# huang-yh/GaussianFormer

Measured on AMD Instinct MI355X. Metric: Gaussians/sec splatted into 200×200×16×18 voxel grid (fwd), higher is better.
Workload: dtype f32

## Files before the change

### gaussianformer_amd/csrc/splat_bwd_mfma.hip

```cpp
#include <algorithm>


#include "gf_common.hpp"
#include "splat_mfma.hpp"

#ifndef GF_TIMELINE
#define GF_TIMELINE 0
#endif

namespace gf {

constexpr int kBwdBigTableAt = kLongWords, kBwdBigTable = (kBwdBigCap - kBwdBigTableAt - 1) / 3;
static_assert(kBwdBigTableAt >= kWRow && kBwdBigTable >= 64, "the table sits past the layout words in use");

struct BwdMArgs {
    const float *pts;
    const float *records;
    const uint2 *boxes;
    const unsigned long long *bitmask;
    const float *out_grad;
    float *rows;
    float *means_grad, *opa_grad, *sem_grad, *cov_grad;
    const uint32_t *state;
    uint32_t *tile_counters;
    const uint32_t *gen_word;
    const uint32_t *row_first;
    const uint32_t *wave_total;
    const uint32_t *lists, *list_len;
    const uint32_t *lists_bad;
    int P, N, nwords, nrow, H, W, D, nsx, nsy;
    int gate;
    int records_asserted;
    unsigned long long *timeline;
    uint32_t *big_table;
    uint32_t m_ps, m_nsy;
    uint32_t cap;
};

static_assert(kBwdList == 256, "kMList");
constexpr int kMList = kBwdList;
constexpr int kMQCap = 128;
constexpr int kMPitch16 = 136;
constexpr int kMDlDwords = kC * kMPitch16;
static_assert(128 * kC <= kMDlDwords, "the 128 fp32 rows land in the same area before they are split");
constexpr int kMFirstAt = 1536 + 3 * kMList + kMDlDwords + kMQCap;
constexpr int kMLdsDwords = kMFirstAt + 64;
constexpr int kMRowAt = 768;
static_assert(kMRowAt + 2 * kWRow <= 1536 + 3 * kMList, "the bitmask row fits over the slot's upper half and the list");
static_assert(3 * kMList <= kMRowAt, "the dense-word compaction borrows the lower half of the record slot");
static_assert(kMLdsDwords * 4 <= 20480, "eight single-wave workgroups per CU");

__device__ __forceinline__ void split16(const f32x16 &d, H8 (&hi)[2], H8 (&lo)[2])
{
#pragma unroll
    for (int q = 0; q < 16; q += 2) {
        const float w0 = d[q], w1 = d[q + 1];
        const fp16x2 h = __builtin_amdgcn_cvt_pkrtz(w0, w1);
        float q0, q1;
        asm("v_fma_mix_f32 %0, %1, -1.0, %2 op_sel_hi:[1,0,0]" : "=v"(q0) : "v"(h), "v"(w0));
        asm("v_fma_mix_f32 %0, %1, -1.0, %2 op_sel:[1,0,0] op_sel_hi:[1,0,0]" : "=v"(q1) : "v"(h), "v"(w1));
        hi[q >> 3].p[(q & 7) >> 1] = h;
        lo[q >> 3].p[(q & 7) >> 1] = __builtin_amdgcn_cvt_pkrtz(q0, q1);
    }
}

struct BwdSetupArgs {
    float *means_grad, *opa_grad, *sem_grad, *cov_grad;
    const uint32_t *wave_total, *row_local;
    uint32_t *row_first;
    uint32_t *gen_word;
    const uint32_t *state;
    uint32_t cap;
    int P;
};

__global__ __launch_bounds__(256) void gf_splat_bwd_setup_kernel(BwdSetupArgs a)
{
    if (!on_matrix_cores(a.state[kStateNotDense], a.state[kStatePath])) return;
    if (records_still_there(a.state, a.gen_word)) return;
    const size_t i0 = (size_t)blockIdx.x * 256 + threadIdx.x, stride = (size_t)gridDim.x * 256;
    for (size_t i = i0; i < (size_t)kC * a.P; i += stride) a.sem_grad[i] = 0.f;
    for (size_t i = i0; i < (size_t)6 * a.P; i += stride) a.cov_grad[i] = 0.f;
    for (size_t i = i0; i < (size_t)3 * a.P; i += stride) a.means_grad[i] = 0.f;
    for (size_t i = i0; i < (size_t)a.P; i += stride) a.opa_grad[i] = 0.f;
    const int nblk = (a.P + 255) >> 8;
    if ((int)blockIdx.x >= nblk) return;
    __shared__ uint32_t s_sum[4];
    const int tid = threadIdx.x, w0 = 4 * (int)blockIdx.x, nw = (a.P + 63) >> 6;
    const int g = 256 * (int)blockIdx.x + tid;
    const uint32_t local = g < a.P ? a.row_local[g] : 0u;
    uint32_t before = 0u;
    for (int w = tid; w < w0; w += 256) before += a.wave_total[w] & 0x7FFFFFFFu;
#pragma unroll
    for (int off = 32; off >= 1; off >>= 1) before += (uint32_t)__shfl_xor((int)before, off, 64);
    if ((tid & 63) == 0) s_sum[tid >> 6] = before;
    __syncthreads();
    uint32_t base = s_sum[0] + s_sum[1] + s_sum[2] + s_sum[3];
    const int wv = tid >> 6;
    uint32_t mine = 0u;
    for (int k = 0; k < 4; ++k) {
        const uint32_t t = w0 + k < nw ? (a.wave_total[w0 + k] & 0x7FFFFFFFu) : 0u;
        if (k < wv) base += t;
        if (k == wv) mine = t;
    }
    if (g < a.P) a.row_first[g] = (unsigned long long)base + mine <= (unsigned long long)a.cap ? base + local : 0xFFFFFFFFu;
}

__device__ __forceinline__ void zero_big_gaussians(const BwdMArgs &a, int lane)
{
    const int nw = (a.P + 63) >> 6;
    constexpr int kPer = (kWRow + 63) / 64;
    static_assert(kPer == 10, "operand list below");
    int nbig = 0;
    for (int kb = 0; 64 * kb < nw; kb += kPer) {
    uint32_t fl[kPer];
#pragma unroll
    for (int k = 0; k < kPer; ++k) fl[k] = a.wave_total[min(64 * (kb + k) + lane, nw - 1)];
    asm volatile("" : "+v"(fl[0]), "+v"(fl[1]), "+v"(fl[2]), "+v"(fl[3]), "+v"(fl[4]), "+v"(fl[5]), "+v"(fl[6]), "+v"(fl[7]), "+v"(fl[8]), "+v"(fl[9]));
#pragma unroll
    for (int k = 0; k < kPer; ++k) {
        const int w0 = 64 * (kb + k);
        const bool f = w0 + lane < nw && (fl[k] >> 31) != 0u;
        unsigned long long m = __builtin_amdgcn_ballot_w64(f);
        while (m) {
            const int w = w0 + __builtin_ctzll(m);
            m &= m - 1;
            const int g = 64 * w + lane;
            bool big_here = false;
            uint32_t first_here = 0u;
            int cnt_here = 0;
            if (g < a.P) {
                const uint2 b = a.boxes[g];
                const bool ne = ux(b.y) > ux(b.x) && uy(b.y) > uy(b.x) && uz(b.y) > uz(b.x);
                const int cnt = !ne ? 0 : (((ux(b.y) - 1) >> 2) - (ux(b.x) >> 2) + 1) * (((uy(b.y) - 1) >> 2) - (uy(b.x) >> 2) + 1) *
                                              (((uz(b.y) - 1) >> 3) - (uz(b.x) >> 3) + 1);
                first_here = a.row_first[g];
                if (cnt > kBwdBigRows && first_here != 0xFFFFFFFFu) {
                    for (int k = 0; k < kC; ++k) a.sem_grad[(size_t)kC * g + k] = 0.f;
                    for (int k = 0; k < 6; ++k) a.cov_grad[6 * (size_t)g + k] = 0.f;
                    for (int k = 0; k < 3; ++k) a.means_grad[3 * (size_t)g + k] = 0.f;
                    a.opa_grad[g] = 0.f;
                    big_here = true;
                    cnt_here = cnt;
                }
            }
            const unsigned long long bm = __builtin_amdgcn_ballot_w64(big_here);
            if (big_here) {
                const int pos = nbig + __builtin_popcountll(bm & ((1ull << lane) - 1ull));
                if (pos < kBwdBigTable) {
                    a.big_table[1 + 3 * pos] = (uint32_t)g;
                    a.big_table[2 + 3 * pos] = first_here;
                    a.big_table[3 + 3 * pos] = (uint32_t)cnt_here;
                }
            }
            nbig += __builtin_popcountll(bm);
        }
    }
    }
    if (lane == 0) a.big_table[0] = nbig <= kBwdBigTable ? (uint32_t)nbig : 0xFFFFFFFFu;
}

template <bool LONG = false>
__global__ __launch_bounds__(64, 2) void gf_splat_bwd_mfma_kernel(BwdMArgs a)
{
    __shared__ __attribute__((aligned(16))) uint32_t s_u[kMLdsDwords];
    float4 *slot = reinterpret_cast<float4 *>(s_u);
    uint32_t *s_lg = s_u + 1536, *s_blo = s_u + 1536 + kMList, *s_bhi = s_u + 1536 + 2 * kMList;
    float *s_dl = reinterpret_cast<float *>(s_u + 1536 + 3 * kMList);
    unsigned long long *s_row = reinterpret_cast<unsigned long long *>(s_u + kMRowAt);
    uint32_t *q_id = s_u + 1536 + 3 * kMList + kMDlDwords;
    _Float16 *s_dh = reinterpret_cast<_Float16 *>(s_dl), *s_dq = s_dh + kC * kMPitch16;

    uint32_t st0 = a.state[kStateNotDense], st1 = a.state[kStatePath], st3 = a.state[kStateGen], st4 = a.state[kStateRows], gen = *a.gen_word;
    uint32_t lbad = a.lists ? *a.lists_bad : 1u;
    asm volatile("" : "+s"(st0), "+s"(st1), "+s"(st3), "+s"(st4), "+s"(gen), "+s"(lbad));
    const bool mc_fwd = on_matrix_cores(st0, st1);
    const bool still_there = st3 == gen && (st4 & kRowsReady) != 0u;
    if (a.gate && !mc_fwd) return;
    if (a.records_asserted && !still_there) return;

    const int lane = threadIdx.x;
    if (blockIdx.x == 0) zero_big_gaussians(a, lane);
    const int n_ = lane & 31, h_ = lane >> 5;
    typedef _Float16 half2_t __attribute__((ext_vector_type(2)));
    const int xcd = (int)(blockIdx.x & 7u);
    const int per_super = 4 * ((a.D + 7) >> 3);
    const int per_xcd = ((a.nsx * a.nsy + 7) >> 3) * per_super;
    const uint32_t m_ps = a.m_ps, m_nsy = a.m_nsy;

    cfloat_t cp = (cfloat_t)(uintptr_t)a.pts;
    const double p0x = cp[0], p0y = cp[1], p0z = cp[2];
    const double sx = a.H > 1 ? (double)cp[3 * (size_t)a.W * a.D] - p0x : 1.0;
    const double sy = a.W > 1 ? (double)cp[3 * (size_t)a.D + 1] - p0y : 1.0;
    const double sz = a.D > 1 ? (double)cp[3 + 2] - p0z : 1.0;

    auto request_records_at = [&](int qh, int start, int count) {
        const uint32_t id = q_id[(qh + start + (n_ < count ? n_ : 0)) & (kMQCap - 1)];
        const char *rec = reinterpret_cast<const char *>(a.records + (size_t)id * kRecDwords);
        const int o3 = (3 + 2 * h_) * 16, o4 = (4 + 2 * h_) * 16, o5 = 7 * 16;
        char *dst = reinterpret_cast<char *>(slot);
        __builtin_amdgcn_global_load_lds((gptr)(rec), (lptr)(dst), 16, 0, 0);
        __builtin_amdgcn_global_load_lds((gptr)(rec + 16), (lptr)(dst + 1024), 16, 0, 0);
        __builtin_amdgcn_global_load_lds((gptr)(rec + 32), (lptr)(dst + 2048), 16, 0, 0);
        __builtin_amdgcn_global_load_lds((gptr)(rec + o3), (lptr)(dst + 3072), 16, 0, 0);
        __builtin_amdgcn_global_load_lds((gptr)(rec + o4), (lptr)(dst + 4096), 16, 0, 0);
        __builtin_amdgcn_global_load_lds((gptr)(rec + o5), (lptr)(dst + 5120), 16, 0, 0);
        __builtin_amdgcn_global_load_lds((gptr)(a.row_first + id), (lptr)(s_u + kMFirstAt), 4, 0, 0);
    };
    auto request_row = [&](const unsigned long long *bm, int wl) {
        for (int i = 0; 128 * i < a.nrow; ++i)
            if (128 * i + 2 * wl < a.nrow)
                __builtin_amdgcn_global_load_lds((gptr)(bm + 128 * i + 2 * wl), (lptr)(s_row + 128 * i), 16, 0, 0);
    };

    const bool dl_by16 = (a.D & 1) == 0;
    const size_t dl_last = (size_t)a.N * kC - (dl_by16 ? 4 : 1);
    const bool use_lists = a.lists && still_there && (LONG || lbad == 0u);
    auto request_unit = [&](int s_, int Xw_, int Y0_, int Zw_) {
        int wl = lane;
        asm volatile("" : "+v"(wl));
        if (use_lists) {
            const int pstride = LONG ? kBwdPubLong : kMList;
            const uint32_t *src = a.lists + (size_t)s_ * (3 * pstride) + 4 * wl;
#pragma unroll
            for (int k = 0; k < 3; ++k)
                __builtin_amdgcn_global_load_lds((gptr)(src + pstride * k), (lptr)(s_lg + kMList * k), 16, 0, 0);
        } else if (!LONG) {
            request_row(a.bitmask + (size_t)s_ * a.nrow, wl);
        }
        const int per_col = dl_by16 ? 36 : 144, step_off = dl_by16 ? 28 : 64, step_col = dl_by16 ? 1 : 0, fl = dl_by16 ? 4 : 1;
        int col = wl >= per_col ? 1 : 0, off = wl - col * per_col;
        const int nreq = dl_by16 ? 9 : 36;
#pragma nounroll
        for (int i = 0; i < nreq; ++i) {
            const int cx = Xw_ + (col >> 2), cy = Y0_ + (col & 3);
            const bool ok = cx < a.H && cy < a.W;
            const size_t vox = ok ? ((size_t)cx * a.W + cy) * a.D + Zw_ : 0;
            const size_t fo = min(vox * kC + (size_t)(off * fl), dl_last);
            const float *src = a.out_grad + fo;
            if (dl_by16) __builtin_amdgcn_global_load_lds((gptr)src, (lptr)(s_dl + 256 * i), 16, 0, 0);
            else __builtin_amdgcn_global_load_lds((gptr)src, (lptr)(s_dl + 64 * i), 4, 0, 0);
            col += step_col; off += step_off;
            if (off >= per_col) { off -= per_col; col += 1; }
        }
    };

    uint32_t *ctr = a.tile_counters + 64 * xcd;
    const int nchunk = (a.nwords + 63) >> 6;
    int local = (int)(blockIdx.x >> 3);
    while (true) {
        const int logical = local;
        const int qs = (int)__umulhi((uint32_t)logical, m_ps);
        if (!(local < per_xcd && 8 * qs + xcd < a.nsx * a.nsy)) break;
        uint32_t claimed = 0u;
        const int s = 8 * qs + xcd, r = logical - qs * per_super;
        const int srow = a.nsy == 1 ? s : (int)__umulhi((uint32_t)s, m_nsy), scol = s - srow * a.nsy;
        const int Xw = srow * kSuper + 4 * (r & 1), Y0 = scol * kSuper + 4 * ((r >> 1) & 1), Zw = 8 * (r >> 2);
        if (Xw < a.H && Y0 < a.W) {
#if GF_TIMELINE
            unsigned long long tl[8] = {(unsigned long long)wall_clock64(), 0, 0, 0, 0, 0, 0, 0};
#endif
            const uint32_t published_len = use_lists ? a.list_len[s] : 0u;
            request_unit(s, Xw, Y0, Zw);
            if (dl_by16) asm volatile("s_waitcnt vmcnt(9)" ::: "memory");
            else asm volatile("s_waitcnt vmcnt(36)" ::: "memory");
#if GF_TIMELINE
            tl[1] = wall_clock64();
#endif
            int list_len = 0, qlen = 0, qhead = 0, npend = 0;
            int c = 0, sg = 0;
            bool have_boxes = false;
            const bool pub_unit = LONG ? (use_lists && published_len != 0xFFFFFFFFu) : use_lists;
            int pub_done = 0;
            bool pub_fetch = false;
            if (pub_unit) {
                list_len = min((int)(LONG ? published_len : (published_len & 0xFFFFu)), kMList);
                c = nchunk;
                have_boxes = true;
            } else if (!LONG) {
                constexpr int kWDense = kMList;
                uint32_t *s_dw = s_u;
                unsigned long long *s_db = reinterpret_cast<unsigned long long *>(s_u + kWDense);
                constexpr int kWPer = (kWRow + 63) / 64;
                const int kw = nchunk;
                unsigned long long wd[kWPer];
                int mine = 0;
                int wlane = lane;
                asm volatile("" : "+v"(wlane));
                const int wbase = kw * wlane;
#pragma unroll
                for (int k = 0; k < kWPer; ++k) wd[k] = s_row[min(wbase + k, kWRow - 1)];
                static_assert(kWPer == 10, "operand list below");
                asm volatile("" : "+v"(wd[0]), "+v"(wd[1]), "+v"(wd[2]), "+v"(wd[3]), "+v"(wd[4]), "+v"(wd[5]), "+v"(wd[6]), "+v"(wd[7]),
                             "+v"(wd[8]), "+v"(wd[9]));
#pragma unroll
                for (int k = 0; k < kWPer; ++k) {
                    const int w = wbase + k;
                    wd[k] = (k < kw && w < a.nwords) ? wd[k] : 0ull;
                    mine += wd[k] != 0ull ? 1 : 0;
                }
                const int incl_nz = wave_incl_scan_dpp(mine);
                const int nd = __builtin_amdgcn_readlane(incl_nz, 63);
                if (nd <= kWDense) {
                    int p = incl_nz - mine;
#pragma unroll
                    for (int k = 0; k < kWPer; ++k) {
                        if (wd[k] != 0ull) {
                            s_dw[p] = (uint32_t)(wbase + k);
                            s_db[p] = wd[k];
                            ++p;
                        }
                    }
                    __builtin_amdgcn_fence(__ATOMIC_ACQ_REL, "wavefront");
                    __builtin_amdgcn_wave_barrier();
                    int tot = 0;
                    bool fits = true;
                    auto extract = [&](unsigned long long bits, uint32_t id0, int pos) {
                        if (bits) {
                            s_lg[pos++] = id0 + (uint32_t)__builtin_ctzll(bits);
                            bits &= bits - 1;
                        }
                        while (bits) {
                            const int j = __builtin_ctzll(bits);
                            bits &= bits - 1;
                            s_lg[pos++] = id0 + (uint32_t)j;
                        }
                    };
                    if (nd <= 192) {
                        unsigned long long bb[3];
                        uint32_t ii[3];
                        int cn[3], in_[3], tt[3];
#pragma unroll
                        for (int q = 0; q < 3; ++q) {
                            bb[q] = s_db[64 * q + lane];
                            ii[q] = s_dw[64 * q + lane];
                        }
                        asm volatile("" : "+v"(bb[0]), "+v"(bb[1]), "+v"(bb[2]), "+v"(ii[0]), "+v"(ii[1]), "+v"(ii[2]));
#pragma unroll
                        for (int q = 0; q < 3; ++q) {
                            bb[q] = 64 * q + lane < nd ? bb[q] : 0ull;
                            ii[q] *= 64u;
                            cn[q] = __builtin_popcountll(bb[q]);
                        }
#pragma unroll
                        for (int q = 0; q < 3; ++q) in_[q] = wave_incl_scan_dpp(cn[q]);
#pragma unroll
                        for (int q = 0; q < 3; ++q) tt[q] = __builtin_amdgcn_readlane(in_[q], 63);
                        tot = tt[0] + tt[1] + tt[2];
                        if (tot <= kMList) {
                            extract(bb[0], ii[0], in_[0] - cn[0]);
                            extract(bb[1], ii[1], tt[0] + in_[1] - cn[1]);
                            extract(bb[2], ii[2], tt[0] + tt[1] + in_[2] - cn[2]);
                        } else {
                            fits = false;
                        }
                    } else {
                        for (int d0 = 0; d0 < nd; d0 += 64) {
                            const int i = d0 + lane;
                            const unsigned long long bits = i < nd ? s_db[i] : 0ull;
                            const uint32_t id0 = (i < nd ? s_dw[i] : 0u) * 64u;
                            const int cnt = __builtin_popcountll(bits);
                            const int incl = wave_incl_scan_dpp(cnt);
                            const int t = __builtin_amdgcn_readlane(incl, 63);
                            if (tot + t > kMList) {
                                fits = false;
                                break;
                            }
                            extract(bits, id0, tot + incl - cnt);
                            tot += t;
                        }
                    }
                    if (fits) {
                        list_len = tot;
                        c = nchunk;
                    }
                }
            }
            const unsigned long long *bm_row = a.bitmask + (size_t)s * a.nrow;
#if GF_TIMELINE
            tl[2] = wall_clock64();
#endif
            __builtin_amdgcn_fence(__ATOMIC_ACQ_REL, "wavefront");
            __builtin_amdgcn_wave_barrier();
            asm volatile("s_waitcnt vmcnt(0)" ::: "memory");
            float dmax = 0.f;
            float v[2 * kC];
            {
                int wl = lane;
                asm volatile("" : "+v"(wl));
                const int ly_ = (wl >> 3) & 3, z_ = wl & 7;
#pragma unroll
                for (int half = 0; half < 2; ++half) {
                    const int lx_ = (wl >> 5) + 2 * half;
                    const bool ok = Xw + lx_ < a.H && Y0 + ly_ < a.W && Zw + z_ < a.D;
                    const float *rowp = s_dl + (64 * half + wl) * kC;
                    const float4 q0 = *reinterpret_cast<const float4 *>(rowp), q1 = *reinterpret_cast<const float4 *>(rowp + 4);
                    const float4 q2 = *reinterpret_cast<const float4 *>(rowp + 8), q3 = *reinterpret_cast<const float4 *>(rowp + 12);
                    const float2 q4 = *reinterpret_cast<const float2 *>(rowp + 16);
                    const float w[kC] = {q0.x, q0.y, q0.z, q0.w, q1.x, q1.y, q1.z, q1.w, q2.x, q2.y, q2.z, q2.w, q3.x, q3.y, q3.z, q3.w, q4.x, q4.y};
#pragma unroll
                    for (int ch = 0; ch < kC; ++ch) v[2 * ch + half] = ok ? w[ch] : 0.f;
                }
#pragma unroll
                for (int k = 0; k < 2 * kC; ++k) dmax = fmaxf(dmax, fabsf(v[k]));
#pragma unroll
                for (int d = 32; d >= 1; d >>= 1) dmax = fmaxf(dmax, __shfl_xor(dmax, d, 64));
            }
            const int dex = min(254, max(5, (int)((__float_as_uint(dmax) >> 23) & 255u)));
            const float dscale = dmax > 0.f ? __uint_as_float((uint32_t)(258 - dex) << 23) : 1.f;
            const int dshift = dmax > 0.f ? dex - 131 : 0;
            {
                __builtin_amdgcn_fence(__ATOMIC_ACQ_REL, "wavefront");
                __builtin_amdgcn_wave_barrier();
                int wl = lane;
                asm volatile("" : "+v"(wl));
                const int colv = 32 * (2 * ((wl >> 2) & 1)) + 16 * ((wl >> 5) & 1) + 4 * ((wl >> 3) & 3) + (wl & 3);
                _Float16 *ph = s_dh + colv, *pq = s_dq + colv;
#pragma unroll
                for (int ch = 0; ch < kC; ++ch) {
                    const float x0 = v[2 * ch] * dscale, x1 = v[2 * ch + 1] * dscale;
                    const fp16x2 hh = __builtin_amdgcn_cvt_pkrtz(x0, x1);
                    float q0, q1;
                    asm("v_fma_mix_f32 %0, %1, -1.0, %2 op_sel_hi:[1,0,0]" : "=v"(q0) : "v"(hh), "v"(x0));
                    asm("v_fma_mix_f32 %0, %1, -1.0, %2 op_sel:[1,0,0] op_sel_hi:[1,0,0]" : "=v"(q1) : "v"(hh), "v"(x1));
                    const fp16x2 ll = __builtin_amdgcn_cvt_pkrtz(q0, q1);
                    ph[ch * kMPitch16] = hh[0]; ph[ch * kMPitch16 + 32] = hh[1];
                    pq[ch * kMPitch16] = ll[0]; pq[ch * kMPitch16 + 32] = ll[1];
                }
                __builtin_amdgcn_fence(__ATOMIC_ACQ_REL, "wavefront");
                __builtin_amdgcn_wave_barrier();
            }
            int n = n_, h = h_;
            asm volatile("" : "+v"(n), "+v"(h));
            h8 phi[4], hotv[2];
        #pragma unroll
            for (int b = 0; b < 4; ++b) {
                const float ux_ = (float)(2 * (b & 1) + (n >> 4)) - 1.5f, uy_ = (float)((n >> 2) & 3) - 1.5f,
                            uz_ = (float)(4 * (b >> 1) + (n & 3)) - 3.5f;
                const float m0[8] = {1.f, ux_, uy_, uz_, ux_ * ux_, 0.f, 0.f, 0.f};
                const float m1[8] = {uy_ * uy_, uz_ * uz_, ux_ * uy_, uy_ * uz_, ux_ * uz_, 0.f, 0.f, 0.f};
        #pragma unroll
                for (int j = 0; j < 8; ++j) phi[b][j] = (_Float16)(h ? m1[j] : m0[j]);
            }
        #pragma unroll
            for (int k = 0; k < 2; ++k) {
                const int lx = 2 * k + (n >> 4), ly = (n >> 2) & 3, zz = 4 * k + (n & 3);
        #pragma unroll
                for (int j = 0; j < 8; ++j) hotv[k][j] = (_Float16)((h ? zz == j : (j < 4 ? lx == j : ly == j - 4)) ? 1.f : 0.f);
            }
            
            half2_t xy2[4][2], z2[2][2];
            {
                const int mono = (n & 4) ? -1 : ((n & 3) + 4 * (n >> 3));
                const int pa[10] = {0, 1, 0, 0, 2, 0, 0, 1, 0, 1}, pb[10] = {0, 0, 1, 0, 0, 2, 0, 1, 1, 0}, pc[10] = {0, 0, 0, 1, 0, 0, 2, 0, 1, 1};
                int ea = 0, eb = 0, ec = 0;
        #pragma unroll
                for (int m = 0; m < 10; ++m) {
                    ea = mono == m ? pa[m] : ea; eb = mono == m ? pb[m] : eb; ec = mono == m ? pc[m] : ec;
                }
                const bool valid_row = mono >= 0 && mono < 10;
                auto pw = [](float x, int e) { return e == 0 ? 1.f : (e == 1 ? x : x * x); };
        #pragma unroll
                for (int t = 0; t < 4; ++t)
        #pragma unroll
                    for (int jy = 0; jy < 2; ++jy) {
                        const float v = valid_row ? pw((float)t - 1.5f, ea) * pw((float)(h + 2 * jy) - 1.5f, eb) : 0.f;
                        xy2[t][jy] = (half2_t){(_Float16)v, (_Float16)v};
                    }
        #pragma unroll
                for (int bz = 0; bz < 2; ++bz)
        #pragma unroll
                    for (int zp = 0; zp < 2; ++zp)
                        z2[bz][zp] = (half2_t){(_Float16)pw((float)(4 * bz + 2 * zp) - 3.5f, ec), (_Float16)pw((float)(4 * bz + 2 * zp + 1) - 3.5f, ec)};
            }
            const double Cx = p0x + ((double)Xw + 1.5) * sx, Cy = p0y + ((double)Y0 + 1.5) * sy, Cz = p0z + ((double)Zw + 3.5) * sz;
            bool have_next = false;
            bool stores_behind = false;
#if GF_TIMELINE
            asm volatile("s_waitcnt lgkmcnt(0)" ::: "memory");
            tl[3] = wall_clock64();
#endif
            while (true) {
                bool last = false;
                if (LONG && pub_unit) {
                    if (pub_fetch) {
                        int wl = lane;
                        asm volatile("" : "+v"(wl));
                        const int e0 = min(pub_done + 4 * wl, kBwdPubLong - 4);
                        const uint32_t *src = a.lists + (size_t)s * (3 * kBwdPubLong) + e0;
#pragma unroll
                        for (int k = 0; k < 3; ++k)
                            __builtin_amdgcn_global_load_lds((gptr)(src + kBwdPubLong * k), (lptr)(s_lg + kMList * k), 16, 0, 0);
                        asm volatile("s_waitcnt vmcnt(0)" ::: "memory");
                        list_len = min((int)published_len - pub_done, kMList);
                        have_boxes = true;
                    }
                    pub_done += list_len;
                    last = pub_done >= (int)published_len;
                    pub_fetch = true;
                }
                while (!(LONG && pub_unit)) {
                    if (c >= nchunk) {
                        last = true;
                        break;
                    }
                    const int w = 64 * c + lane;
                    unsigned long long bits = w < a.nwords ? bm_row[w] : 0ull;
                    const int cnt = __builtin_popcountll(bits);
                    const int incl = wave_incl_scan_dpp(cnt);
                    const int total = __builtin_amdgcn_readlane(incl, 63);
                    int pos = -1;
                    if (total <= kMList) {
                        if (list_len + total > kMList) break;
                        pos = list_len + incl - cnt;
                        list_len += total;
                        ++c;
                    } else {
                        static_assert(4 * 64 <= kMList, "a lane group of four words fits the empty list");
                        bool full = false;
                        for (; sg < 16; ++sg) {
                            const int e1 = __builtin_amdgcn_readlane(incl, 4 * sg + 3);
                            const int e0 = sg ? __builtin_amdgcn_readlane(incl, 4 * sg - 1) : 0;
                            if (list_len + (e1 - e0) > kMList) {
                                full = true;
                                break;
                            }
                            if ((lane >> 2) == sg) pos = list_len + (incl - cnt) - e0;
                            list_len += e1 - e0;
                        }
                        if (!full) {
                            sg = 0;
                            ++c;
                        }
                        if (pos >= 0) {
                            const uint32_t id0 = (uint32_t)w * 64u;
                            while (bits) {
                                const int j = __builtin_ctzll(bits);
                                bits &= bits - 1;
                                s_lg[pos++] = id0 + (uint32_t)j;
                            }
                        }
                        if (full) break;
                        continue;
                    }
                    const uint32_t id0 = (uint32_t)w * 64u;
                    while (bits) {
                        const int j = __builtin_ctzll(bits);
                        bits &= bits - 1;
                        s_lg[pos++] = id0 + (uint32_t)j;
                    }
                }
                __builtin_amdgcn_fence(__ATOMIC_ACQ_REL, "wavefront");
                __builtin_amdgcn_wave_barrier();
                if (!have_boxes) {
                    for (int b0 = 0; b0 < list_len; b0 += 64) {
                        const uint32_t id = s_lg[min(b0 + lane, list_len - 1)];
                        __builtin_amdgcn_global_load_lds((gptr)(&a.boxes[id].x), (lptr)(s_blo + b0), 4, 0, 0);
                        __builtin_amdgcn_global_load_lds((gptr)(&a.boxes[id].y), (lptr)(s_bhi + b0), 4, 0, 0);
                    }
                    asm volatile("s_waitcnt vmcnt(0)" ::: "memory");
                }
                have_boxes = false;
                stores_behind = false;
                for (int base = 0; base < list_len || (last && base == 0); base += 64) {
                    const int i = base + lane;
                    const int ic = min(i, max(list_len - 1, 0));
                    const uint32_t eg = s_lg[ic];
                    const uint32_t blo = s_blo[ic], bhi = s_bhi[ic];
                    const bool hit = i < list_len && ux(blo) < Xw + 4 && ux(bhi) > Xw && uy(blo) < Y0 + 4 && uy(bhi) > Y0 &&
                                     uz(blo) < Zw + 8 && uz(bhi) > Zw;
                    const unsigned long long todo = __builtin_amdgcn_ballot_w64(hit);
                    if (hit) q_id[(qhead + qlen + (int)mbcnt(todo)) & (kMQCap - 1)] = eg;
                    qlen += __builtin_popcountll(todo);
                    const bool final_batch = last && base + 64 >= list_len;
                    while (true) {
                        if (npend == 0) {
                            if (!(qlen >= 32 || (final_batch && qlen > 0))) break;
                            npend = min(qlen, 32);
                            __builtin_amdgcn_fence(__ATOMIC_ACQ_REL, "wavefront");
                            __builtin_amdgcn_wave_barrier();
                            request_records_at(qhead, 0, npend);
                            stores_behind = false;
                        }
                        const int avail = qlen - npend;
                        if (!(avail >= 32 || final_batch)) break;
                        const int qn = npend;
                        if (stores_behind) asm volatile("s_waitcnt vmcnt(6)" ::: "memory");
                        else asm volatile("s_waitcnt vmcnt(0)" ::: "memory");
#if GF_TIMELINE
                        if (!tl[4]) tl[4] = wall_clock64();
                        tl[7] += 1;
#endif
                        const bool live = n < qn;
                        const float4 r0 = slot[lane], r1 = slot[64 + lane], r2 = slot[128 + lane];
                        const float4 e0 = slot[192 + lane], e1 = slot[256 + lane], e2 = slot[320 + lane];
                        const uint32_t my_id = q_id[(qhead + (live ? n : 0)) & (kMQCap - 1)];
                        const uint32_t first = s_u[kMFirstAt + lane];
                        __builtin_amdgcn_fence(__ATOMIC_ACQ_REL, "wavefront");
                        __builtin_amdgcn_wave_barrier();
                        const int nnext = min(avail, 32);
                        if (nnext > 0) request_records_at(qhead, qn, nnext);
                        const bool last_group = final_batch && nnext == 0;
                        if (last_group && lane == 0)
                            asm volatile("global_atomic_add %0, %1, %2, off sc0" : "=v"(claimed) : "v"(ctr), "v"(1u) : "memory");
                        H8 b0h, b0l, b1h, b1l;
                        int sshift = 0;
                        {
                            float sv[10] = {e0.x, e0.y, e0.z, e0.w, e1.x, e1.y, e1.z, e1.w, e2.x, e2.y};
                            float smax = 0.f;
#pragma unroll
                            for (int j = 0; j < 10; ++j) {
                                sv[j] = live ? sv[j] : 0.f;
                                smax = fmaxf(smax, fabsf(sv[j]));
                            }
                            smax = fmaxf(smax, __builtin_bit_cast(float, __builtin_amdgcn_ds_bpermute((lane ^ 32) << 2, __builtin_bit_cast(int, smax))));
                            const int sex = min(252, (int)((__float_as_uint(smax) >> 23) & 255u));
                            const float sscale = smax > 0.f ? __uint_as_float((uint32_t)(253 - sex) << 23) : 1.f;
                            sshift = smax > 0.f ? sex - 126 : 0;
#pragma unroll
                            for (int j = 0; j < 10; ++j) sv[j] *= sscale;
                            if (h) { sv[8] = 0.f; sv[9] = 0.f; }
                            const fp16x2 zz = __builtin_amdgcn_cvt_pkrtz(0.f, 0.f);
#pragma unroll
                            for (int j = 0; j < 10; j += 2) {
                                const fp16x2 hh = __builtin_amdgcn_cvt_pkrtz(sv[j], sv[j + 1]);
                                float q0, q1;
                                asm("v_fma_mix_f32 %0, %1, -1.0, %2 op_sel_hi:[1,0,0]" : "=v"(q0) : "v"(hh), "v"(sv[j]));
                                asm("v_fma_mix_f32 %0, %1, -1.0, %2 op_sel:[1,0,0] op_sel_hi:[1,0,0]" : "=v"(q1) : "v"(hh), "v"(sv[j + 1]));
                                const fp16x2 ll = __builtin_amdgcn_cvt_pkrtz(q0, q1);
                                if (j < 8) { b0h.p[j >> 1] = hh; b0l.p[j >> 1] = ll; }
                                else { b1h.p[0] = hh; b1l.p[0] = ll; }
                            }
#pragma unroll
                            for (int j = 1; j < 4; ++j) { b1h.p[j] = zz; b1l.p[j] = zz; }
                            b1h.p[1] = b1l.p[0]; b1h.p[2] = b1h.p[0];
                        }
                        H8 t1, t2, t3;
                        double ex = 0, ey = 0, ez = 0;
                        {
                            const double L = 1.4426950408889634074;
                            const double c0 = r1.x, c1 = r1.y, c2 = r1.z, c3 = r1.w, c4 = r2.x, c5 = r2.y;
                            double th[5];
                            if (h == 0) {
                                ex = Cx - (double)r0.x; ey = Cy - (double)r0.y; ez = Cz - (double)r0.z;
                                const double gx = c0 * ex + c3 * ey + c5 * ez, gy = c3 * ex + c1 * ey + c4 * ez, gz = c5 * ex + c4 * ey + c2 * ez;
                                th[0] = -0.5 * L * (ex * gx + ey * gy + ez * gz);
                                th[1] = -L * sx * gx; th[2] = -L * sy * gy; th[3] = -L * sz * gz;
                                th[4] = -0.5 * L * sx * sx * c0;
                            } else {
                                th[0] = -0.5 * L * sy * sy * c1; th[1] = -0.5 * L * sz * sz * c2;
                                th[2] = -L * sx * sy * c3; th[3] = -L * sy * sz * c4; th[4] = -L * sx * sz * c5;
                            }
#pragma unroll
                            for (int j = 0; j < 5; ++j) split3(live ? th[j] : 0.0, t1.e[j], t2.e[j], t3.e[j]);
#pragma unroll
                            for (int j = 5; j < 8; ++j) { t1.e[j] = (_Float16)0.f; t2.e[j] = (_Float16)0.f; t3.e[j] = (_Float16)0.f; }
                        }
                        H8 tb;
                        {
                            const uint32_t glo = __float_as_uint(r2.z), ghi = __float_as_uint(r2.w);
                            const int x0 = ux(glo) - Xw, x1 = ux(ghi) - Xw, y0 = uy(glo) - Y0, y1 = uy(ghi) - Y0;
                            const int z0 = uz(glo) - Zw, z1 = uz(ghi) - Zw;
#pragma unroll
                            for (int j = 0; j < 8; ++j) {
                                const bool in = h ? (j >= z0 && j < z1) : (j < 4 ? (j >= x0 && j < x1) : (j - 4 >= y0 && j - 4 < y1));
                                tb.e[j] = (_Float16)((in && live) ? 0.f : -32768.f);
                            }
                        }
                        f32x16 mom, dsm;
#pragma unroll
                        for (int q = 0; q < 16; ++q) { mom[q] = 0.f; dsm[q] = 0.f; }
#pragma unroll
                        for (int b = 0; b < 4; ++b) {
                            typedef int i32x4 __attribute__((ext_vector_type(4)));
                            const i32x4 hv0 = __builtin_bit_cast(i32x4, hotv[0]), hv1 = __builtin_bit_cast(i32x4, hotv[1]);
                            i32x4 hs;
#pragma unroll
                            for (int j = 0; j < 4; ++j) hs[j] = (b == 0) ? hv0[j] : (b == 3) ? hv1[j] : ((b == 1) == (h != 0)) ? hv0[j] : hv1[j];
                            H8 hot;
                            hot.v = __builtin_bit_cast(h8, hs);
                            f32x16 T;
#pragma unroll
                            for (int q = 0; q < 16; ++q) T[q] = 0.f;
                            {
                                const _Float16 *dh = s_dh + (8 * h) * kMPitch16 + 32 * b + n, *dq = s_dq + (8 * h) * kMPitch16 + 32 * b + n;
                                H8 a0h, a0l, a1h, a1l;
#pragma unroll
                                for (int j = 0; j < 8; ++j) { a0h.e[j] = dh[j * kMPitch16]; a0l.e[j] = dq[j * kMPitch16]; }
                                const _Float16 *dh1 = s_dh + 16 * kMPitch16 + 32 * b + n, *dq1 = s_dq + 16 * kMPitch16 + 32 * b + n;
                                const _Float16 zero16 = (_Float16)0.f;
                                a1h.e[0] = h ? zero16 : dh1[0]; a1h.e[1] = h ? zero16 : dh1[kMPitch16];
                                a1l.e[0] = h ? zero16 : dq1[0]; a1l.e[1] = h ? zero16 : dq1[kMPitch16];
#pragma unroll
                                for (int j = 2; j < 8; ++j) { a1h.e[j] = zero16; a1l.e[j] = zero16; }
                                T = __builtin_amdgcn_mfma_f32_32x32x16_f16(a0l.v, b0h.v, T, 0, 0, 0);
                                T = __builtin_amdgcn_mfma_f32_32x32x16_f16(a0h.v, b0l.v, T, 0, 0, 0);
                                a1h.p[1] = a1h.p[0]; a1h.p[2] = a1l.p[0];
                                T = __builtin_amdgcn_mfma_f32_32x32x16_f16(a1h.v, b1h.v, T, 0, 0, 0);
                                T = __builtin_amdgcn_mfma_f32_32x32x16_f16(a0h.v, b0h.v, T, 0, 0, 0);
                            }
                            f32x16 d;
#pragma unroll
                            for (int q = 0; q < 16; ++q) d[q] = 0.f;
                            d = __builtin_amdgcn_mfma_f32_32x32x16_f16(phi[b], t3.v, d, 0, 0, 0);
                            d = __builtin_amdgcn_mfma_f32_32x32x16_f16(phi[b], t2.v, d, 0, 0, 0);
                            d = __builtin_amdgcn_mfma_f32_32x32x16_f16(phi[b], t1.v, d, 0, 0, 0);
                            d = __builtin_amdgcn_mfma_f32_32x32x16_f16(hot.v, tb.v, d, 0, 0, 0);
                            f32x16 e, K;
#pragma unroll
                            for (int q = 0; q < 16; ++q) e[q] = __builtin_amdgcn_exp2f(d[q]);
#pragma unroll
                            for (int q = 0; q < 16; ++q) K[q] = e[q] * T[q];
                            H8 eh[2], el[2], kh_[2], kl_[2];
                            split16(e, eh, el);
                            split16(K, kh_, kl_);
#pragma unroll
                            for (int kc = 0; kc < 2; ++kc) {
                                union { h8 v; half2_t p[4]; } pt;
                                pt.p[0] = xy2[2 * (b & 1) + kc][0] * z2[b >> 1][0];
                                pt.p[1] = xy2[2 * (b & 1) + kc][0] * z2[b >> 1][1];
                                pt.p[2] = xy2[2 * (b & 1) + kc][1] * z2[b >> 1][0];
                                pt.p[3] = xy2[2 * (b & 1) + kc][1] * z2[b >> 1][1];
                                mom = __builtin_amdgcn_mfma_f32_32x32x16_f16(pt.v, kl_[kc].v, mom, 0, 0, 0);
                                mom = __builtin_amdgcn_mfma_f32_32x32x16_f16(pt.v, kh_[kc].v, mom, 0, 0, 0);
                                const int dco = min(n, kC - 1) * kMPitch16 + 32 * b + 16 * kc + 4 * h;
                                union { h8 v; uint2 u[2]; } ah, al;
                                ah.u[0] = *reinterpret_cast<const uint2 *>(s_dh + dco); ah.u[1] = *reinterpret_cast<const uint2 *>(s_dh + dco + 8);
                                al.u[0] = *reinterpret_cast<const uint2 *>(s_dq + dco); al.u[1] = *reinterpret_cast<const uint2 *>(s_dq + dco + 8);
                                dsm = __builtin_amdgcn_mfma_f32_32x32x16_f16(al.v, eh[kc].v, dsm, 0, 0, 0);
                                dsm = __builtin_amdgcn_mfma_f32_32x32x16_f16(ah.v, el[kc].v, dsm, 0, 0, 0);
                                dsm = __builtin_amdgcn_mfma_f32_32x32x16_f16(ah.v, eh[kc].v, dsm, 0, 0, 0);
                            }
                            __builtin_amdgcn_sched_barrier(0);
                        }
                        {
                            const float opa = r0.w;
                            const double fs = __builtin_ldexp(1.0, dshift);
                            const double fm = __builtin_ldexp(1.0, dshift + sshift);
                            float o[24];
                            if (h == 0) {
                                const double S0 = mom[0] * fm, S1x = mom[1] * fm, S1y = mom[2] * fm, S1z = mom[3] * fm;
                                const double Sxx = mom[4] * fm, Syy = mom[5] * fm, Szz = mom[6] * fm, Sxy = mom[7] * fm, Syz = mom[8] * fm, Sxz = mom[9] * fm;
                                const double D1x = -(ex * S0 + sx * S1x), D1y = -(ey * S0 + sy * S1y), D1z = -(ez * S0 + sz * S1z);
                                const double D2xx = ex * ex * S0 + 2.0 * ex * sx * S1x + sx * sx * Sxx;
                                const double D2yy = ey * ey * S0 + 2.0 * ey * sy * S1y + sy * sy * Syy;
                                const double D2zz = ez * ez * S0 + 2.0 * ez * sz * S1z + sz * sz * Szz;
                                const double D2xy = ex * ey * S0 + ex * sy * S1y + ey * sx * S1x + sx * sy * Sxy;
                                const double D2yz = ey * ez * S0 + ey * sz * S1z + ez * sy * S1y + sy * sz * Syz;
                                const double D2xz = ex * ez * S0 + ex * sz * S1z + ez * sx * S1x + sx * sz * Sxz;
                                const double c0 = r1.x, c1 = r1.y, c2 = r1.z, c3 = r1.w, c4 = r2.x, c5 = r2.y, po = opa;
                                o[0] = (float)(po * dsm[0] * fs); o[1] = (float)(po * dsm[1] * fs); o[2] = (float)(po * dsm[2] * fs); o[3] = (float)(po * dsm[3] * fs);
                                o[4] = (float)(po * dsm[4] * fs); o[5] = (float)(po * dsm[5] * fs); o[6] = (float)(po * dsm[6] * fs); o[7] = (float)(po * dsm[7] * fs);
                                o[8] = (float)(po * dsm[8] * fs); o[9] = (float)(po * dsm[9] * fs);
                                o[10] = (float)(-0.5 * po * D2xx); o[11] = (float)(-0.5 * po * D2yy); o[12] = (float)(-0.5 * po * D2zz);
                                o[13] = (float)(-po * D2xy); o[14] = (float)(-po * D2yz); o[15] = (float)(-po * D2xz);
                                o[16] = (float)(-po * (c0 * D1x + c3 * D1y + c5 * D1z));
                                o[17] = (float)(-po * (c3 * D1x + c1 * D1y + c4 * D1z));
                                o[18] = (float)(-po * (c5 * D1x + c4 * D1y + c2 * D1z));
                                o[19] = (float)S0;
                            } else {
                                const double po = opa;
#pragma unroll
                                for (int k = 0; k < 8; ++k) o[k] = (float)(po * dsm[k] * fs);
#pragma unroll
                                for (int k = 8; k < 20; ++k) o[k] = 0.f;
                            }
                            const uint32_t glo = __float_as_uint(r2.z), ghi = __float_as_uint(r2.w);
                            const int bx0 = ux(glo) >> 2, by0 = uy(glo) >> 2, bz0 = uz(glo) >> 3;
                            const int nby = ((uy(ghi) - 1) >> 2) - by0 + 1, nbz = ((uz(ghi) - 1) >> 3) - bz0 + 1;
                            const int nbx = ((ux(ghi) - 1) >> 2) - bx0 + 1;
                            const int idx = (((Xw >> 2) - bx0) * nby + ((Y0 >> 2) - by0)) * nbz + ((Zw >> 3) - bz0);
                            const bool has_row = live && first != 0xFFFFFFFFu && (unsigned long long)first + (unsigned long long)(uint32_t)idx < (unsigned long long)a.cap;
                            if (has_row) {
                                float4 *row = reinterpret_cast<float4 *>(a.rows + ((size_t)first + (size_t)idx) * kBwdRowDwords);
                                row[h] = make_float4(o[0], o[1], o[2], o[3]);
                                row[2 + h] = make_float4(o[4], o[5], o[6], o[7]);
                                if (h == 0) {
                                    row[4] = make_float4(o[8], o[9], o[10], o[11]);
                                    row[5] = make_float4(o[12], o[13], o[14], o[15]);
                                    row[6] = make_float4(o[16], o[17], o[18], o[19]);
                                    row[7] = make_float4(__uint_as_float(my_id), __uint_as_float((uint32_t)(nbx * nby * nbz)), __uint_as_float((uint32_t)idx), 0.f);
                                }
                            } else if (live) {
                                float *sg_ = a.sem_grad + (size_t)kC * my_id;
                                if (h == 0) {
#pragma unroll
                                    for (int k = 0; k < 4; ++k) { unsafeAtomicAdd(sg_ + k, o[k]); unsafeAtomicAdd(sg_ + 8 + k, o[4 + k]); }
                                    unsafeAtomicAdd(sg_ + 16, o[8]); unsafeAtomicAdd(sg_ + 17, o[9]);
#pragma unroll
                                    for (int k = 0; k < 6; ++k) unsafeAtomicAdd(a.cov_grad + 6 * (size_t)my_id + k, o[10 + k]);
#pragma unroll
                                    for (int k = 0; k < 3; ++k) unsafeAtomicAdd(a.means_grad + 3 * (size_t)my_id + k, o[16 + k]);
                                    unsafeAtomicAdd(a.opa_grad + my_id, o[19]);
                                } else {
#pragma unroll
                                    for (int k = 0; k < 4; ++k) { unsafeAtomicAdd(sg_ + 4 + k, o[k]); unsafeAtomicAdd(sg_ + 12 + k, o[4 + k]); }
                                }
                            }
                        }
                        stores_behind = nnext > 0;
                        have_next = have_next || last_group;
                        qhead = (qhead + qn) & (kMQCap - 1);
                        qlen -= qn;
                        npend = nnext;
                    }
                }
                if (last) break;
                list_len = 0;
            }
#if GF_TIMELINE
            tl[5] = wall_clock64();
#endif
            if (!have_next) {
                if (lane == 0) asm volatile("global_atomic_add %0, %1, %2, off sc0" : "=v"(claimed) : "v"(ctr), "v"(1u) : "memory");
                asm volatile("s_waitcnt vmcnt(0)" : "+v"(claimed)::"memory");
            } else {
                asm volatile("s_waitcnt vmcnt(6)" : "+v"(claimed)::"memory");
            }
            asm volatile("s_waitcnt lgkmcnt(0)" ::: "memory");
#if GF_TIMELINE
            tl[6] = wall_clock64();
            if (a.timeline && lane == 0)
#pragma unroll
                for (int k = 0; k < 8; ++k) a.timeline[8 * (size_t)logical + k] = tl[k];
#endif
        } else {
            if (lane == 0) asm volatile("global_atomic_add %0, %1, %2, off sc0" : "=v"(claimed) : "v"(ctr), "v"(1u) : "memory");
            asm volatile("s_waitcnt vmcnt(0)" : "+v"(claimed)::"memory");
        }
        local = __builtin_amdgcn_readfirstlane((int)claimed);
    }
}

struct BwdRowsArgs {
    const float *records;
    float *rows;
    float *means_grad, *opa_grad, *sem_grad, *cov_grad;
    const uint32_t *wave_total;
    const uint32_t *row_first;
    uint32_t *gen_word;
    const uint32_t *big_table;
    uint32_t *unit_counters;
    const uint32_t *state;
    uint32_t counter_init;
    int P, gate, ngauss_blocks, records_asserted;
};

__device__ __forceinline__ void bwd_store_column(const BwdRowsArgs &a, int g, int col, float v)
{
    float *dst = col < 18 ? a.sem_grad + (size_t)kC * g + col
               : col < 24 ? a.cov_grad + 6 * (size_t)g + (col - 18)
               : col < 27 ? a.means_grad + 3 * (size_t)g + (col - 24)
               : col == 27 ? a.opa_grad + g : nullptr;
    if (dst) *dst = v;
}
__device__ __forceinline__ void bwd_add_column(const BwdRowsArgs &a, int g, int col, float v)
{
    float *dst = col < 18 ? a.sem_grad + (size_t)kC * g + col
               : col < 24 ? a.cov_grad + 6 * (size_t)g + (col - 18)
               : col < 27 ? a.means_grad + 3 * (size_t)g + (col - 24)
               : a.opa_grad + g;
    unsafeAtomicAdd(dst, v);
}

__global__ __launch_bounds__(256) void gf_splat_bwd_rows_kernel(BwdRowsArgs a)
{
    const int tid = threadIdx.x;
    const bool gauss_range = (int)blockIdx.x < a.ngauss_blocks;
    const int g_own = min((int)blockIdx.x * 32 + (tid >> 3), a.P - 1);
    uint32_t st0 = a.state[kStateNotDense], st1 = a.state[kStatePath], st3 = a.state[kStateGen], st4 = a.state[kStateRows], gen = *a.gen_word;
    uint32_t tab_n = gauss_range ? 0u : a.big_table[0], tab_w = gauss_range ? 0u : a.big_table[1 + min(tid, 3 * 64 - 1)];
    uint32_t first_own = a.row_first[gauss_range ? g_own : 0];
    float4 rec2_own = *reinterpret_cast<const float4 *>(a.records + (size_t)(gauss_range ? g_own : 0) * kRecDwords + 8);
    asm volatile("" : "+s"(st0), "+s"(st1), "+s"(st3), "+s"(st4), "+s"(gen), "+v"(first_own), "+v"(rec2_own.z), "+v"(rec2_own.w), "+v"(tab_n), "+v"(tab_w));
    const bool mc = on_matrix_cores(st0, st1), still_there = records_still_there(st3, st4, gen);
    if (a.gate == 1 && !mc) return;
    const bool bad = (a.gate == 2 && !mc) || (a.records_asserted && !still_there);
    if (!bad && blockIdx.x == 0) {
        if (tid < 8) a.unit_counters[64 * tid] = a.counter_init;
        if (!a.records_asserted && tid == 0 && !still_there) *a.gen_word = gen + 1u;
    }
    auto rows_of_box = [&](uint32_t glo, uint32_t ghi) -> int {
        if (!(ux(ghi) > ux(glo) && uy(ghi) > uy(glo) && uz(ghi) > uz(glo))) return 0;
        return (((ux(ghi) - 1) >> 2) - (ux(glo) >> 2) + 1) * (((uy(ghi) - 1) >> 2) - (uy(glo) >> 2) + 1) *
               (((uz(ghi) - 1) >> 3) - (uz(glo) >> 3) + 1);
    };
    auto box_rows = [&](int g) -> int {
        const float4 r2 = *reinterpret_cast<const float4 *>(a.records + (size_t)g * kRecDwords + 8);
        const uint32_t glo = __float_as_uint(r2.z), ghi = __float_as_uint(r2.w);
        if (!(ux(ghi) > ux(glo) && uy(ghi) > uy(glo) && uz(ghi) > uz(glo))) return 0;
        return (((ux(ghi) - 1) >> 2) - (ux(glo) >> 2) + 1) * (((uy(ghi) - 1) >> 2) - (uy(glo) >> 2) + 1) *
               (((uz(ghi) - 1) >> 3) - (uz(glo) >> 3) + 1);
    };
    if ((int)blockIdx.x < a.ngauss_blocks) {
        constexpr int kRowsInFlight = 20;
        const int g = blockIdx.x * 32 + (tid >> 3), c4 = 4 * (tid & 7);
        if (g >= a.P) return;
        float4 acc = make_float4(0.f, 0.f, 0.f, 0.f);
        if (bad) {
            acc.x = acc.y = acc.z = acc.w = __uint_as_float(0x7fc00000u);
        } else {
            const uint32_t first = first_own;
            const int cnt = rows_of_box(__float_as_uint(rec2_own.z), __float_as_uint(rec2_own.w));
            if (cnt > 0 && (first == 0xFFFFFFFFu || cnt > kBwdBigRows)) return;
            const float *base = a.rows + (size_t)first * kBwdRowDwords + c4;
            for (int r = 0; r < cnt; r += kRowsInFlight) {
                float4 v[kRowsInFlight];
#pragma unroll
                for (int k = 0; k < kRowsInFlight; ++k) v[k] = *reinterpret_cast<const float4 *>(base + (size_t)min(r + k, cnt - 1) * kBwdRowDwords);
#pragma unroll
                for (int k = 0; k < kRowsInFlight; ++k) {
                    const bool in = r + k < cnt;
                    acc.x += in ? v[k].x : 0.f; acc.y += in ? v[k].y : 0.f; acc.z += in ? v[k].z : 0.f; acc.w += in ? v[k].w : 0.f;
                }
            }
        }
        bwd_store_column(a, g, c4, acc.x);
        bwd_store_column(a, g, c4 + 1, acc.y);
        bwd_store_column(a, g, c4 + 2, acc.z);
        bwd_store_column(a, g, c4 + 3, acc.w);
        return;
    }
    if (bad) return;
    __shared__ __attribute__((aligned(16))) float s_part[32][32];
    __shared__ int s_wave[kLongWords], s_cnt[64];
    __shared__ uint32_t s_first[64];
    __shared__ int s_nwave;
    __shared__ uint32_t s_tab[3 * 64];
    int item = (int)blockIdx.x - a.ngauss_blocks;
    const int stride = (int)gridDim.x - a.ngauss_blocks;
    const int lg = tid >> 3, c4 = 4 * (tid & 7);
    auto sum_rows = [&](const float *src, int n, size_t pitch) -> float {
        float4 acc = make_float4(0.f, 0.f, 0.f, 0.f);
        for (int r = lg; r < n; r += 64) {
            const float4 v0 = *reinterpret_cast<const float4 *>(src + (size_t)r * pitch);
            const float4 v1 = *reinterpret_cast<const float4 *>(src + (size_t)min(r + 32, n - 1) * pitch);
            const bool in1 = r + 32 < n;
            acc.x += v0.x; acc.y += v0.y; acc.z += v0.z; acc.w += v0.w;
            acc.x += in1 ? v1.x : 0.f; acc.y += in1 ? v1.y : 0.f; acc.z += in1 ? v1.z : 0.f; acc.w += in1 ? v1.w : 0.f;
        }
        __syncthreads();
        *reinterpret_cast<float4 *>(&s_part[lg][c4]) = acc;
        __syncthreads();
        float t = 0.f;
        if (tid < 32) {
#pragma unroll
            for (int k = 0; k < 32; ++k) t += s_part[k][tid];
        }
        return t;
    };
    tab_n = (uint32_t)__builtin_amdgcn_readfirstlane((int)tab_n);
    if (tab_n <= 64u) {
        if (tid < 3 * 64) s_tab[tid] = tab_w;
        __syncthreads();
        for (uint32_t j = 0; j < tab_n; ++j) {
            const int g = (int)s_tab[3 * j], cnt = (int)s_tab[3 * j + 2];
            const float *grows = a.rows + (size_t)s_tab[3 * j + 1] * kBwdRowDwords;
            const int parts = (cnt + 63) / 64;
            while (item < parts) {
                const int r0 = item * 64;
                const float t = sum_rows(grows + (size_t)r0 * kBwdRowDwords + c4, min(cnt - r0, 64), kBwdRowDwords);
                if (tid < 28) bwd_add_column(a, g, tid, t);
                item += stride;
            }
            item -= parts;
        }
        return;
    }
    const int nw = (a.P + 63) >> 6;
    {
        uint32_t wt[kLongWords / 256];
#pragma unroll
        for (int k = 0; k < kLongWords / 256; ++k) wt[k] = a.wave_total[min(tid + 256 * k, nw - 1)];
#pragma unroll
        for (int k = 0; k < kLongWords / 256; ++k) s_wave[tid + 256 * k] = (int)(wt[k] >> 31);
    }
    __syncthreads();
    if (tid < 64) {
        int n = 0;
        bool fs[kLongWords / 64];
#pragma unroll
        for (int k = 0; k < kLongWords / 64; ++k) fs[k] = 64 * k + tid < nw && s_wave[64 * k + tid] != 0;
        __builtin_amdgcn_fence(__ATOMIC_ACQ_REL, "wavefront");
        __builtin_amdgcn_wave_barrier();
#pragma unroll
        for (int k = 0; k < kLongWords / 64; ++k) {
            const int w0 = 64 * k;
            const bool f = fs[k];
            const unsigned long long m = __builtin_amdgcn_ballot_w64(f);
            if (f) s_wave[n + __builtin_popcountll(m & ((1ull << tid) - 1ull))] = w0 + tid;
            n += __builtin_popcountll(m);
        }
        if (tid == 0) s_nwave = n;
    }
    __syncthreads();
    const int nflag = s_nwave;
    for (int e = 0; e < nflag; ++e) {
        __syncthreads();
        if (tid < 64) {
            const int gq = 64 * s_wave[e] + tid;
            const uint32_t first = gq < a.P ? a.row_first[gq] : 0xFFFFFFFFu;
            const int cnt = gq < a.P ? box_rows(gq) : 0;
            s_cnt[tid] = first == 0xFFFFFFFFu ? 0 : cnt;
            s_first[tid] = first;
        }
        __syncthreads();
        for (int j = 0; j < 64; ++j) {
            const int cnt = s_cnt[j];
            if (cnt <= kBwdBigRows) continue;
            const int g = 64 * s_wave[e] + j;
            const float *grows = a.rows + (size_t)s_first[j] * kBwdRowDwords;
            const int parts = (cnt + 63) / 64;
            while (item < parts) {
                const int r0 = item * 64;
                const float t = sum_rows(grows + (size_t)r0 * kBwdRowDwords + c4, min(cnt - r0, 64), kBwdRowDwords);
                if (tid < 28) bwd_add_column(a, g, tid, t);
                item += stride;
            }
            item -= parts;
        }
    }
}

}

namespace gf {

static unsigned long long *g_bwd_timeline = nullptr;

void launch_splat_backward_mfma(const SplatInputs &in, const SplatGrads &g, const uint32_t *state, const SplatWorkspace &ws, int gate,
                                int records_asserted, hipStream_t stream)
{
    uint32_t *gen_word = ws.flags + kGenWord;
    if (!records_asserted) {
        launch_prep_for_backward(in, state, ws, stream);
        BwdSetupArgs z{g.means_grad, g.opa_grad, g.sem_grad, g.cov_grad, ws.bwd_wave_total, ws.bwd_row_local, ws.bwd_row_first, gen_word, state,
                       ws.bwd_cap, in.P};
        hipLaunchKernelGGL(gf_splat_bwd_setup_kernel, dim3(std::max((in.P + 255) / 256, std::min(1024, (kC * in.P + 255) / 256))), dim3(256), 0,
                           stream, z);
    }
    const int grid = splat_unit_grid(splat_units(ws.nsuper, in.D));
    BwdMArgs a;
    a.pts = in.pts; a.records = ws.records; a.boxes = ws.boxes; a.bitmask = ws.bitmask; a.out_grad = g.out_grad; a.rows = ws.bwd_rows;
    a.means_grad = g.means_grad; a.opa_grad = g.opa_grad; a.sem_grad = g.sem_grad; a.cov_grad = g.cov_grad; a.state = state;
    a.tile_counters = ws.flags + kBwdCounters; a.gen_word = gen_word; a.row_first = ws.bwd_row_first; a.wave_total = ws.bwd_wave_total;
    a.big_table = ws.bwd_wave_total + kBwdBigTableAt;
    a.lists = ws.bwd_lists; a.list_len = ws.bwd_list_len; a.lists_bad = ws.flags + kListsBad;
    a.P = in.P; a.N = in.N; a.nwords = ws.nwords; a.nrow = ws.nrow; a.H = in.H; a.W = in.W; a.D = in.D; a.nsx = ws.nsx; a.nsy = ws.nsy;
    a.gate = gate ? 1 : 0; a.records_asserted = records_asserted;
    a.timeline = g_bwd_timeline;
    a.cap = ws.bwd_cap;
    a.m_ps = ceil_recip32(splat_units(1, in.D)); a.m_nsy = ceil_recip32(ws.nsy);
    if (ws.nrow > kWRow) hipLaunchKernelGGL(gf_splat_bwd_mfma_kernel<true>, dim3(grid), dim3(64), 0, stream, a);
    else hipLaunchKernelGGL(gf_splat_bwd_mfma_kernel<false>, dim3(grid), dim3(64), 0, stream, a);
    BwdRowsArgs r{ws.records, ws.bwd_rows, g.means_grad, g.opa_grad, g.sem_grad, g.cov_grad, ws.bwd_wave_total, ws.bwd_row_first, gen_word,
                  ws.bwd_wave_total + kBwdBigTableAt, ws.flags + kBwdCounters, state, (uint32_t)(grid / 8), in.P, gate, (in.P + 31) / 32, records_asserted};
    hipLaunchKernelGGL(gf_splat_bwd_rows_kernel, dim3(r.ngauss_blocks + 256), dim3(256), 0, stream, r);
}

}

extern "C" void gf_debug_set_bwd_timeline(void *dev_ptr) { gf::g_bwd_timeline = (unsigned long long *)dev_ptr; }
```

Baseline: 752.1 million.

## Trim backward record loads and use transposed LDS reads for MFMA operands

Changes the backward splat kernel's record fetch from six to four global-to-LDS loads per lane by offsetting each half-wave by 64 bytes, and remaps the slot reads accordingly. Replaces strided per-element fp16 LDS gathers of the dL operand with ds_read_tr16_b64 transposed reads. Drops the live-masking of scale and theta values. The intent is less load traffic and fewer LDS instructions per group, but the vmcnt accounting and slot remapping must stay consistent, and dead lanes now carry stale data.

Measured after the change: 757.5 million (median of 4 runs). About the same (+0.7%).

```diff
diff --git a/gaussianformer_amd/csrc/splat_bwd_mfma.hip b/gaussianformer_amd/csrc/splat_bwd_mfma.hip
--- a/gaussianformer_amd/csrc/splat_bwd_mfma.hip
+++ b/gaussianformer_amd/csrc/splat_bwd_mfma.hip
@@ -40,6 +40,7 @@
 static_assert(kBwdList == 256, "kMList");
 constexpr int kMList = kBwdList;
 constexpr int kMQCap = 128;
+constexpr int kGroupStores = 6;
 constexpr int kMPitch16 = 136;
 constexpr int kMDlDwords = kC * kMPitch16;
 static_assert(128 * kC <= kMDlDwords, "the 128 fp32 rows land in the same area before they are split");
@@ -197,14 +198,12 @@
     auto request_records_at = [&](int qh, int start, int count) {
         const uint32_t id = q_id[(qh + start + (n_ < count ? n_ : 0)) & (kMQCap - 1)];
         const char *rec = reinterpret_cast<const char *>(a.records + (size_t)id * kRecDwords);
-        const int o3 = (3 + 2 * h_) * 16, o4 = (4 + 2 * h_) * 16, o5 = 7 * 16;
         char *dst = reinterpret_cast<char *>(slot);
+        rec += 64 * h_;
         __builtin_amdgcn_global_load_lds((gptr)(rec), (lptr)(dst), 16, 0, 0);
         __builtin_amdgcn_global_load_lds((gptr)(rec + 16), (lptr)(dst + 1024), 16, 0, 0);
         __builtin_amdgcn_global_load_lds((gptr)(rec + 32), (lptr)(dst + 2048), 16, 0, 0);
-        __builtin_amdgcn_global_load_lds((gptr)(rec + o3), (lptr)(dst + 3072), 16, 0, 0);
-        __builtin_amdgcn_global_load_lds((gptr)(rec + o4), (lptr)(dst + 4096), 16, 0, 0);
-        __builtin_amdgcn_global_load_lds((gptr)(rec + o5), (lptr)(dst + 5120), 16, 0, 0);
+        __builtin_amdgcn_global_load_lds((gptr)(rec + 48), (lptr)(dst + 3072), 16, 0, 0);
         __builtin_amdgcn_global_load_lds((gptr)(a.row_first + id), (lptr)(s_u + kMFirstAt), 4, 0, 0);
     };
     auto request_row = [&](const unsigned long long *bm, int wl) {
@@ -585,15 +584,15 @@
                         const int avail = qlen - npend;
                         if (!(avail >= 32 || final_batch)) break;
                         const int qn = npend;
-                        if (stores_behind) asm volatile("s_waitcnt vmcnt(6)" ::: "memory");
+                        if (stores_behind) asm volatile("s_waitcnt vmcnt(%0)" ::"n"(kGroupStores) : "memory");
                         else asm volatile("s_waitcnt vmcnt(0)" ::: "memory");
 #if GF_TIMELINE
                         if (!tl[4]) tl[4] = wall_clock64();
                         tl[7] += 1;
 #endif
                         const bool live = n < qn;
-                        const float4 r0 = slot[lane], r1 = slot[64 + lane], r2 = slot[128 + lane];
-                        const float4 e0 = slot[192 + lane], e1 = slot[256 + lane], e2 = slot[320 + lane];
+                        const float4 r0 = slot[n], r1 = slot[64 + n], r2 = slot[128 + n];
+                        const float4 e0 = slot[(h ? 96 : 192) + n], e1 = slot[(h ? 160 : 32) + n], e2 = slot[224 + n];
                         const uint32_t my_id = q_id[(qhead + (live ? n : 0)) & (kMQCap - 1)];
                         const uint32_t first = s_u[kMFirstAt + lane];
                         __builtin_amdgcn_fence(__ATOMIC_ACQ_REL, "wavefront");
@@ -610,7 +609,6 @@
                             float smax = 0.f;
 #pragma unroll
                             for (int j = 0; j < 10; ++j) {
-                                sv[j] = live ? sv[j] : 0.f;
                                 smax = fmaxf(smax, fabsf(sv[j]));
                             }
                             smax = fmaxf(smax, __builtin_bit_cast(float, __builtin_amdgcn_ds_bpermute((lane ^ 32) << 2, __builtin_bit_cast(int, smax))));
@@ -652,7 +650,7 @@
                                 th[2] = -L * sx * sy * c3; th[3] = -L * sy * sz * c4; th[4] = -L * sx * sz * c5;
                             }
 #pragma unroll
-                            for (int j = 0; j < 5; ++j) split3(live ? th[j] : 0.0, t1.e[j], t2.e[j], t3.e[j]);
+                            for (int j = 0; j < 5; ++j) split3(th[j], t1.e[j], t2.e[j], t3.e[j]);
 #pragma unroll
                             for (int j = 5; j < 8; ++j) { t1.e[j] = (_Float16)0.f; t2.e[j] = (_Float16)0.f; t3.e[j] = (_Float16)0.f; }
                         }
@@ -683,16 +681,23 @@
 #pragma unroll
                             for (int q = 0; q < 16; ++q) T[q] = 0.f;
                             {
-                                const _Float16 *dh = s_dh + (8 * h) * kMPitch16 + 32 * b + n, *dq = s_dq + (8 * h) * kMPitch16 + 32 * b + n;
                                 H8 a0h, a0l, a1h, a1l;
-#pragma unroll
-                                for (int j = 0; j < 8; ++j) { a0h.e[j] = dh[j * kMPitch16]; a0l.e[j] = dq[j * kMPitch16]; }
-                                const _Float16 *dh1 = s_dh + 16 * kMPitch16 + 32 * b + n, *dq1 = s_dq + 16 * kMPitch16 + 32 * b + n;
-                                const _Float16 zero16 = (_Float16)0.f;
-                                a1h.e[0] = h ? zero16 : dh1[0]; a1h.e[1] = h ? zero16 : dh1[kMPitch16];
-                                a1l.e[0] = h ? zero16 : dq1[0]; a1l.e[1] = h ? zero16 : dq1[kMPitch16];
-#pragma unroll
-                                for (int j = 2; j < 8; ++j) { a1h.e[j] = zero16; a1l.e[j] = zero16; }
+                                typedef short i16x4 __attribute__((ext_vector_type(4)));
+                                typedef __attribute__((address_space(3))) i16x4 *trptr;
+                                const int tq = (n >> 2) & 3, tcol = 32 * b + (n & 16) + 4 * (n & 3);
+                                const _Float16 *th0 = s_dh + (8 * h + tq) * kMPitch16 + tcol, *th1 = s_dh + (16 + min(tq, 1)) * kMPitch16 + tcol;
+                                constexpr int kLoAt = kC * kMPitch16;
+                                static_assert((kMPitch16 * 2) % 8 == 0 && (kLoAt * 2) % 8 == 0, "8-byte aligned rows");
+                                const uint2 v0 = __builtin_bit_cast(uint2, __builtin_amdgcn_ds_read_tr16_b64_v4i16((trptr)th0));
+                                const uint2 v1 = __builtin_bit_cast(uint2, __builtin_amdgcn_ds_read_tr16_b64_v4i16((trptr)(th0 + 4 * kMPitch16)));
+                                const uint2 w0 = __builtin_bit_cast(uint2, __builtin_amdgcn_ds_read_tr16_b64_v4i16((trptr)(th0 + kLoAt)));
+                                const uint2 w1 = __builtin_bit_cast(uint2, __builtin_amdgcn_ds_read_tr16_b64_v4i16((trptr)(th0 + kLoAt + 4 * kMPitch16)));
+                                const uint2 c1h = __builtin_bit_cast(uint2, __builtin_amdgcn_ds_read_tr16_b64_v4i16((trptr)th1));
+                                const uint2 c1l = __builtin_bit_cast(uint2, __builtin_amdgcn_ds_read_tr16_b64_v4i16((trptr)(th1 + kLoAt)));
+                                a0h.u[0] = v0.x; a0h.u[1] = v0.y; a0h.u[2] = v1.x; a0h.u[3] = v1.y;
+                                a0l.u[0] = w0.x; a0l.u[1] = w0.y; a0l.u[2] = w1.x; a0l.u[3] = w1.y;
+                                a1h.u[0] = h ? 0u : c1h.x; a1l.u[0] = h ? 0u : c1l.x;
+                                a1h.u[1] = 0u; a1h.u[2] = 0u; a1h.u[3] = 0u; a1l.u[1] = 0u; a1l.u[2] = 0u; a1l.u[3] = 0u;
                                 T = __builtin_amdgcn_mfma_f32_32x32x16_f16(a0l.v, b0h.v, T, 0, 0, 0);
                                 T = __builtin_amdgcn_mfma_f32_32x32x16_f16(a0h.v, b0l.v, T, 0, 0, 0);
                                 a1h.p[1] = a1h.p[0]; a1h.p[2] = a1l.p[0];
@@ -772,6 +777,7 @@
                             const int idx = (((Xw >> 2) - bx0) * nby + ((Y0 >> 2) - by0)) * nbz + ((Zw >> 3) - bz0);
                             const bool has_row = live && first != 0xFFFFFFFFu && (unsigned long long)first + (unsigned long long)(uint32_t)idx < (unsigned long long)a.cap;
                             if (has_row) {
+                                static_assert(kGroupStores == 6, "the six stores below");
                                 float4 *row = reinterpret_cast<float4 *>(a.rows + ((size_t)first + (size_t)idx) * kBwdRowDwords);
                                 row[h] = make_float4(o[0], o[1], o[2], o[3]);
                                 row[2 + h] = make_float4(o[4], o[5], o[6], o[7]);
@@ -815,7 +821,7 @@
                 if (lane == 0) asm volatile("global_atomic_add %0, %1, %2, off sc0" : "=v"(claimed) : "v"(ctr), "v"(1u) : "memory");
                 asm volatile("s_waitcnt vmcnt(0)" : "+v"(claimed)::"memory");
             } else {
-                asm volatile("s_waitcnt vmcnt(6)" : "+v"(claimed)::"memory");
+                asm volatile("s_waitcnt vmcnt(%1)" : "+v"(claimed) : "n"(kGroupStores) : "memory");
             }
             asm volatile("s_waitcnt lgkmcnt(0)" ::: "memory");
 #if GF_TIMELINE
```
